# jay-tux/cutrace

Measured on AMD Instinct MI355X. Metric: Mrays/sec (primary+secondary), higher is better.
Workload: dtype f32; 1 GPU; bunny.json@1920x1080 bounces=5 fudge=1e-3, 1 frame(s)/step row-tiled over 1 GPU(s), gather to rank 0; steps_in_flight=1

## Files before the change

cutrace_amd/__init__.py:

```python
import contextlib
import ctypes as C
import os

import numpy as np

from . import _lib
from ._lib import Camera, Light, Material, Object, RenderStats, Rows, SceneDesc, Triangle, Vec3

ROOT = _lib.ROOT

VAR_AUTO = 0
VAR_NO_PREFILTER = 2
VAR_NO_ANYHIT = 4
VAR_NO_CLUSTER = 8
VAR_STATS = 16
VAR_EXACT_POW = 32
VAR_NO_REORDER = 256
VAR_NO_OCC6 = 512
VAR_NO_DIRECT = 1024
VAR_IMAGE_ORDER_FIRST = 2048
VAR_MERGE = 4096
VAR_IGNORE_TRANSPARENT = 8192

RAY_IGNORE_TRANSPARENT = 1
# ... 166 lines not shown
            st = L.ctr_render(self._h, C.c_float(fudge), bounces, C.byref(r), depth.ctypes.data, color.ctypes.data,
                              normal.ctypes.data, C.byref(stats))
            if st:
                raise RuntimeError(f"ctr_render failed ({st}): {L.ctr_last_error().decode()}")
        return dict(depth=depth, color=color, normal=normal, ray_count=int(stats.ray_count),
                    kernel_ms=stats.kernel_ms, total_ms=stats.total_ms, max_depth=float(stats.max_depth),
                    rows=int(stats.rows))

    def render_uv(self, fudge=1e-3, bounces=5, rows=None):
        L = _lib.hip_lib()
        r = make_rows(self.h, rows)
        n = rows_count(self.h, rows)
        depth = np.empty((n, self.w), np.float32)
        color = np.empty((n, self.w, 3), np.float32)
        normal = np.empty((n, self.w, 3), np.float32)
        uv = np.empty((n, self.w, 2), np.float32)
        stats = RenderStats()
        st = L.ctr_render_uv(self._h, C.c_float(fudge), bounces, C.byref(r), depth.ctypes.data, color.ctypes.data,
                             normal.ctypes.data, uv.ctypes.data, C.byref(stats))
        if st:
            raise RuntimeError(f"ctr_render_uv failed ({st}): {L.ctr_last_error().decode()}")
        return dict(depth=depth, color=color, normal=normal, uv=uv, ray_count=int(stats.ray_count),
                    kernel_ms=stats.kernel_ms, total_ms=stats.total_ms, max_depth=float(stats.max_depth), rows=int(stats.rows))

    def render_device(self, d_depth, d_color, d_normal, d_counters=0, stream=0, fudge=1e-3, bounces=5, rows=None, samples=1):
        samples = self._samples(samples)
        L = _lib.hip_lib()
        r = make_rows(self.h, rows)
        if samples != 1:
            st = L.ctr_render_device_aa(self._h, C.c_float(fudge), bounces, samples, C.byref(r), d_depth, d_color, d_normal,
                                        d_counters, stream)
            if st:
                raise RuntimeError(f"ctr_render_device_aa failed ({st}): {L.ctr_last_error().decode()}")
            return
        st = L.ctr_render_device(self._h, C.c_float(fudge), bounces, C.byref(r), d_depth, d_color, d_normal,
                                 d_counters, stream)
        if st:
            raise RuntimeError(f"ctr_render_device failed ({st}): {L.ctr_last_error().decode()}")

    def set_cameras(self, cams):
        arr = (Camera * len(cams))(*cams)
        st = _lib.hip_lib().ctr_scene_set_cameras(self._h, arr, len(cams))
        if st:
            raise RuntimeError(f"ctr_scene_set_cameras failed: {_lib.hip_lib().ctr_last_error().decode()}")
        self.n_cams = len(cams)

    def render_device_batch(self, d_depth, d_color, d_normal, n_frames, frame_stride_px, first_frame=0, d_counters=0,
                            stream=0, fudge=1e-3, bounces=5, rows=None, part_stride=0):
        L = _lib.hip_lib()
        r = make_rows(self.h, rows)
        st = L.ctr_render_device_batch(self._h, C.c_float(fudge), bounces, C.byref(r), first_frame, n_frames,
                                       frame_stride_px, part_stride, d_depth, d_color, d_normal, d_counters, stream)
        if st:
            raise RuntimeError(f"ctr_render_device_batch failed ({st}): {L.ctr_last_error().decode()}")

    def algorithmic_bytes(self, fudge=1e-3, bounces=5, rows=None):
        L = _lib.hip_lib()
        r = make_rows(self.h, rows)
        b = C.c_uint64()
        n = C.c_uint64()
        st = L.ctr_algorithmic_bytes(self._h, C.c_float(fudge), bounces, C.byref(r), C.byref(b), C.byref(n))
        if st:
            raise RuntimeError(f"ctr_algorithmic_bytes failed ({st}): {L.ctr_last_error().decode()}")
        return int(b.value), int(n.value)

    def last_counters(self):
        out = np.zeros(16, np.uint64)
        _lib.hip_lib().ctr_last_counters(self._h, out.ctypes.data)
        return out

    @staticmethod
    def lane_stats(reset=True):
        raw = np.zeros(96, np.uint64)
        if _lib.hip_lib().ctr_debug_lane_stats(raw.ctypes.data, 1 if reset else 0):
            raise RuntimeError("ctr_debug_lane_stats failed")
        c = [int(x) for x in raw]
        trips, live = c[72], c[73]
        out = {"wave_trips": trips, "live_lanes_per_trip": live / trips if trips else None,
               "live_fraction": live / (64.0 * trips) if trips else None,
               "live_fraction_of_in_image_lanes": (live / trips) / (c[75] / c[74]) if trips and c[74] and c[75] else None,
               "trips_by_live_lanes_1_8_to_57_64": c[64:72], "trips_mixing_kinds": c[76], "waves": c[74],
               "merged_walks": c[78], "merged_walks_redone": c[77],
               "shadow_casts_at_meshes": {"wave_casts": c[80], "receivers_all_off_mesh": c[81], "of_those_unoccluded_by_meshes": c[82],
                                          "unoccluded_by_meshes_any_receiver": c[83]}}
        kinds = {}
        for d in range(16):
            for name, base in (("radiance", 0), ("shadow", 16)):
                if c[32 + base + d]:
                    label = "primary" if (name == "radiance" and d == 0) else f"{name}@depth{d}"
                    kinds[label] = {"lanes": c[base + d], "trips": c[32 + base + d],
                                    "lanes_per_trip": c[base + d] / c[32 + base + d]}
        out["by_kind"] = kinds
        return out

    def _torch_device(self):
        import torch
        return torch.device("cuda", self.device)

    def _rays_arg(self, x, what, cols):
        import torch
        dev = self._torch_device()
        if isinstance(x, torch.Tensor):
            if x.device.type != "cpu" and x.device != dev:
                raise ValueError(f"{what}: tensor on {x.device}, the scene lives on {dev}")
        elif isinstance(x, np.ndarray):
            x = torch.from_numpy(x)
        else:
            raise TypeError(f"{what}: expected a torch tensor or a numpy array, got {type(x).__name__}")
        shape_ok = x.dim() == 1 if cols == 0 else (x.dim() == 2 and x.shape[1] == cols)
        if x.dtype != torch.float32 or not shape_ok:
            raise ValueError(f"{what}: expected float32 of shape {'(n,)' if cols == 0 else f'(n, {cols})'}, "
                             f"got {x.dtype} {tuple(x.shape)}")
        return x.to(dev, non_blocking=False).contiguous()

    def _cast(self, q, keep, stream):
        import torch
        q.n_rays = keep[0].shape[0]
        q.d_origin, q.d_dir = keep[0].data_ptr() or None, keep[1].data_ptr() or None
        st = _lib.hip_lib().ctr_cast_rays(self._h, C.byref(q), C.c_void_p(stream.cuda_stream))
        if st:
            raise RuntimeError(f"ctr_cast_rays failed ({st}): {_lib.hip_lib().ctr_last_error().decode()}")

    def _per_ray(self, x, n, what):
        if isinstance(x, (int, float, np.integer, np.floating)):
            return float(x), None
        v = self._rays_arg(x, what, 0)
        if v.shape[0] != n:
            raise ValueError(f"{what}: {v.shape[0]} values for {n} rays")
        return 0.0, v

    def cast_rays(self, origins, dirs, min_t=1e-3, ignore_transparent=False, linear=False, outputs=None, stream=None):
        import torch
        outputs = RAY_OUTPUTS if outputs is None else tuple(outputs)
        bad = [k for k in outputs if k not in RAY_OUTPUTS]
        if bad or not outputs:
            raise ValueError(f"outputs: a non-empty subset of {RAY_OUTPUTS}, got {outputs}")
        dev = self._torch_device()
        with torch.cuda.device(dev), torch.cuda.stream(stream if stream is not None else torch.cuda.current_stream(dev)):
            o = self._rays_arg(origins, "origins", 3)
            d = self._rays_arg(dirs, "dirs", 3)
            n = o.shape[0]
            if d.shape[0] != n:
                raise ValueError(f"dirs: {d.shape[0]} rays for {n} origins")
            q = _lib.RayQuery()
            q.flags = (RAY_IGNORE_TRANSPARENT if ignore_transparent else 0) | (RAY_LINEAR if linear else 0)
            q.min_t, mt = self._per_ray(min_t, n, "min_t")
            q.d_min_t = mt.data_ptr() if mt is not None and n else None
            shapes = {"t": ((n,), torch.float32), "object": ((n,), torch.int32), "prim": ((n,), torch.int32),
                      "point": ((n, 3), torch.float32), "normal": ((n, 3), torch.float32), "uv": ((n, 2), torch.float32)}
            out = {k: torch.empty(*shapes[k][0], dtype=shapes[k][1], device=dev) for k in outputs}
            for k, v in out.items():
                setattr(q, "d_" + k, v.data_ptr() if n else None)
            if n:
                self._cast(q, (o, d, mt), torch.cuda.current_stream(dev))
        return out

    def shadow(self, origins, dirs, max_t, linear=False, stream=None):
        import torch
        dev = self._torch_device()
        with torch.cuda.device(dev), torch.cuda.stream(stream if stream is not None else torch.cuda.current_stream(dev)):
            o = self._rays_arg(origins, "origins", 3)
            d = self._rays_arg(dirs, "dirs", 3)
            n = o.shape[0]
            if d.shape[0] != n:
                raise ValueError(f"dirs: {d.shape[0]} rays for {n} origins")
            q = _lib.RayQuery()
            q.flags = RAY_SHADOW | (RAY_LINEAR if linear else 0)
# ... 171 lines not shown
```

cutrace_amd/csrc/render_kernel.hip:

```cpp
#include <hip/hip_runtime.h>
#include <math.h>
#include <stddef.h>
#include <stdint.h>
#include <stdlib.h>

#include "cutrace_amd.h"
#include "scene_device.h"
#include "bvh.h"

#define CADDR __attribute__((address_space(4)))
#define BALLOT(p) __builtin_amdgcn_ballot_w64(p)
#define HIDE_UNIFORM(x) asm volatile("" : "+v"(x))
#define PIN3(a, b, c) asm volatile("" : "+v"(a), "+v"(b), "+v"(c))
#define INVB(m) __builtin_amdgcn_inverse_ballot_w64(m)
#define FCMP(a, b, pred) __builtin_amdgcn_fcmpf((a), (b), (pred))
enum { FC_OEQ = 1, FC_OGT = 2, FC_OGE = 3, FC_OLT = 4, FC_OLE = 5 };
#define TL_NONE 0x7FFFFFFFu

extern "C" __device__ uint32_t ctr_writelane(uint32_t value, uint32_t lane, uint32_t old) __asm("llvm.amdgcn.writelane.i32");

namespace {

#if defined(CTR_PROFILE)
__device__ unsigned int g_prof[128];
// ... 372 lines not shown
        atomicAdd(&g_lane_stats[64 + ((n_live - 1u) >> 3)], 1ull);
        atomicAdd(&g_lane_stats[72], 1ull);
        atomicAdd(&g_lane_stats[73], (unsigned long long)n_live);
        if (kinds > 1u) atomicAdd(&g_lane_stats[76], 1ull);
        if (first_trip) { atomicAdd(&g_lane_stats[74], 1ull); atomicAdd(&g_lane_stats[75], (unsigned long long)__builtin_popcountll(img_m)); }
      }
    }

    float best = INFINITY;
    int bobj = -1, btri = -1;
    mask_t alive_m = active_m;
    V3 rinv = mk(0, 0, 0);
    bool have_rinv = false;
    V3 ria = mk(0, 0, 0);
    float ria_big = 0.f;
    float cmax = 0.f;
    if (k_has_mesh) {
      CTR_MARK(2);
      ria = mk(fminf(fmaxf(__builtin_amdgcn_rcpf(rd.x), -1e30f), 1e30f),
               fminf(fmaxf(__builtin_amdgcn_rcpf(rd.y), -1e30f), 1e30f),
               fminf(fmaxf(__builtin_amdgcn_rcpf(rd.z), -1e30f), 1e30f));
      ria_big = fmaxf(fmaxf(fabsf(ria.x), fabsf(ria.y)), fabsf(ria.z));
      cmax = fmaxf(fmaxf(fabsf(rd.x), fabsf(rd.y)), fabsf(rd.z));
    }

    TSTAMP(t_loop0);
    TACC(0, t_trip0, t_loop0);
    CTR_MARK(3);
    const bool anyhit_cast = ANYHIT && shadow_cast;
    const bool ign_now = IGNTR && first_trip;
    {
      mask_t live_m = alive_m;
      const float mt_lo = min_t - fabsf(min_t) * 0x1p-21f;
      float lhv = anyhit_cast ? light_dist : best;
      lhv = lhv + fabsf(lhv) * 0x1p-21f;
      float tiny = 1e-37f;
      asm volatile("" : "+v"(tiny));
      auto plane_exact = [&](uint32_t pidx, float num, float den, mask_t need_m, auto site) -> bool {
        CTR_MARK(110 + decltype(site)::value);
        bool retire = false;
        if (INVB(need_m)) {
          const float t0 = num / den;
          if (__builtin_isfinite(t0) && t0 > min_t) {
            if (t0 < best || (t0 == best && (int)pidx < bobj)) {
              best = t0; bobj = (int)pidx; btri = -1;
              if (!anyhit_cast) lhv = t0 + fabsf(t0) * 0x1p-21f;
            }
            if (anyhit_cast && t0 < light_dist) retire = true;
          }
        }
        if (ANYHIT) {
          live_m &= ~BALLOT(retire);
          if (live_m == 0ull) return false;
        }
        return true;
      };
      auto plane_test = [&](uint32_t pidx, float num, float den, auto site) -> bool {
        CTR_MARK(100 + decltype(site)::value);
        const float nump = __uint_as_float(__float_as_uint(num) ^ (__float_as_uint(den) & 0x80000000u));
        const float denp = fabsf(den);
        const mask_t need_m = live_m & ~(FCMP(nump, __builtin_fmaf(mt_lo, denp, -tiny), FC_OLT) |
                                         FCMP(nump, __builtin_fmaf(lhv, denp, tiny), FC_OGT));
        if (need_m == 0ull) return true;
        return plane_exact(pidx, num, den, need_m, site);
      };
      const float2_ rox = {ro.x, ro.x}, roy = {ro.y, ro.y}, roz = {ro.z, ro.z};
      const float2_ rdx = {rd.x, rd.x}, rdy = {rd.y, rd.y}, rdz = {rd.z, rd.z};
      auto num_den = [&](const CADDR DPlanePair &P, float2_ &num, float2_ &den) {
        const float2_ nx = ldpair(P.n[0]), ny = ldpair(P.n[1]), nz = ldpair(P.n[2]);
        const float2_ dx = ldpair(P.p[0]) - rox, dy = ldpair(P.p[1]) - roy, dz = ldpair(P.p[2]) - roz;
        num = (dx * nx + dy * ny) + dz * nz;
        den = (rdx * nx + rdy * ny) + rdz * nz;
      };
      const uint32_t n_recs = k_plane_recs, n_axis = k_axis_recs;
      bool axis_fast = false;
      if (n_axis != 0u && A.fudge >= 1e-30f) {
        CTR_MARK(4);
        const float chk = __builtin_fmaf(ro.x, 4.0f, __builtin_fmaf(ro.y, 4.0f, __builtin_fmaf(ro.z, 4.0f, (rd.x + rd.y) + rd.z))) * 0.0f;
        axis_fast = (alive_m & ~FCMP(chk, 0.0f, FC_OEQ)) == 0ull;
      }
      auto triple_tests = [&](uint32_t i00, uint32_t i01, uint32_t i10, uint32_t i11, uint32_t i20, uint32_t i21, float2_ num0, float2_ den0,
                              float2_ num1, float2_ den1, float2_ num2, float2_ den2, uint32_t tr00, uint32_t tr01, uint32_t tr10,
                              uint32_t tr11, uint32_t tr20, uint32_t tr21) -> bool {
        if (i00 != CTR_PLANE_PAD && !(IGNTR && ign_now && tr00)) { if (!plane_test(i00, num0.x, den0.x, SITE(0))) return false; }
        if (i01 != CTR_PLANE_PAD && !(IGNTR && ign_now && tr01)) { if (!plane_test(i01, num0.y, den0.y, SITE(1))) return false; }
        if (i10 != CTR_PLANE_PAD && !(IGNTR && ign_now && tr10)) { if (!plane_test(i10, num1.x, den1.x, SITE(2))) return false; }
        if (i11 != CTR_PLANE_PAD && !(IGNTR && ign_now && tr11)) { if (!plane_test(i11, num1.y, den1.y, SITE(3))) return false; }
        if (i20 != CTR_PLANE_PAD && !(IGNTR && ign_now && tr20)) { if (!plane_test(i20, num2.x, den2.x, SITE(4))) return false; }
        if (i21 != CTR_PLANE_PAD && !(IGNTR && ign_now && tr21)) { if (!plane_test(i21, num2.y, den2.y, SITE(5))) return false; }
        return true;
      };
      uint32_t p = 0;
      bool more = true;
      if (k_head_axis && axis_fast) {
        CTR_MARK(59);
        auto pr = [&](int k) -> float2_ { const float2_ v = {__uint_as_float(hd_ax[2 * k]), __uint_as_float(hd_ax[2 * k + 1])}; return v; };
        const float2_ nx = pr(1), ny = pr(3), nz = pr(5);
        uint32_t tr00 = 0u, tr01 = 0u, tr10 = 0u, tr11 = 0u, tr20 = 0u, tr21 = 0u;
        if (IGNTR && ign_now) {
          tr00 = AK->head.ax_transparent[0]; tr01 = AK->head.ax_transparent[1]; tr10 = AK->head.ax_transparent[2];
          tr11 = AK->head.ax_transparent[3]; tr20 = AK->head.ax_transparent[4]; tr21 = AK->head.ax_transparent[5];
        }
        p = 3u;
        more = triple_tests(hd_ax[12], hd_ax[13], hd_ax[14], hd_ax[15], hd_ix[0], hd_ix[1], (pr(0) - rox) * nx, rdx * nx, (pr(2) - roy) * ny,
                            rdy * ny, (pr(4) - roz) * nz, rdz * nz, tr00, tr01, tr10, tr11, tr20, tr21);
      }
      while (more && p < n_recs) {
        if (n_recs - p >= 3u) {
          float2_ num0, den0, num1, den1, num2, den2;
          uint32_t i00, i01, i10, i11, i20, i21;
          uint32_t tr00 = 0u, tr01 = 0u, tr10 = 0u, tr11 = 0u, tr20 = 0u, tr21 = 0u;
          const CADDR DPlanePair &P0 = k_planes[p], &P1 = k_planes[p + 1], &P2 = k_planes[p + 2];
          i00 = P0.index[0]; i01 = P0.index[1]; i10 = P1.index[0]; i11 = P1.index[1]; i20 = P2.index[0]; i21 = P2.index[1];
          if (IGNTR && ign_now) {
            tr00 = P0.transparent[0]; tr01 = P0.transparent[1]; tr10 = P1.transparent[0];
            tr11 = P1.transparent[1]; tr20 = P2.transparent[0]; tr21 = P2.transparent[1];
          }
          if (p < n_axis && axis_fast) {
            CTR_MARK(5);
            const float2_ nx = ldpair(P0.n[0]), ny = ldpair(P1.n[1]), nz = ldpair(P2.n[2]);
            num0 = (ldpair(P0.p[0]) - rox) * nx; den0 = rdx * nx;
            num1 = (ldpair(P1.p[1]) - roy) * ny; den1 = rdy * ny;
            num2 = (ldpair(P2.p[2]) - roz) * nz; den2 = rdz * nz;
          } else {
            CTR_MARK(6);
            num_den(P0, num0, den0);
            num_den(P1, num1, den1);
            num_den(P2, num2, den2);
          }
          p += 3;
          if (!triple_tests(i00, i01, i10, i11, i20, i21, num0, den0, num1, den1, num2, den2, tr00, tr01, tr10, tr11, tr20, tr21)) break;
        } else {
          const CADDR DPlanePair &P0 = k_planes[p];
          CTR_MARK(7);
          float2_ num0, den0;
          num_den(P0, num0, den0);
          const uint32_t i00 = P0.index[0], i01 = P0.index[1];
          p += 1;
          if (!(IGNTR && ign_now && P0.transparent[0])) { if (!plane_test(i00, num0.x, den0.x, SITE(6))) break; }
          if (i01 != CTR_PLANE_PAD && !(IGNTR && ign_now && P0.transparent[1])) {
            if (!plane_test(i01, num0.y, den0.y, SITE(7))) break;
          }
        }
      }
      if (ANYHIT) alive_m = live_m;
    }
    TSTAMP(t_planes1);
    TACC(1, t_loop0, t_planes1);
    CTR_MARK(8);
    V3 sph_d = mk(0, 0, 0);
    float sph_dd = 0.f;
    bool sph_have = false;
    for (uint32_t oi = 0; oi < k_n_oloop; ++oi) {
      if (ANYHIT) {
        if (alive_m == 0ull) break;
      }
      const CADDR DObj &O = AK->oloop[oi];
      const uint32_t i = O.index;
      const uint32_t type = O.type;
      if (IGNTR && ign_now && __float_as_uint(O.f[7]) != 0u) continue;
      CTR_MARK(9);
      bool ok = false;
      float cand = INFINITY;
      int ctri = -1;
      if (type == CTR_OBJ_SPHERE) {
        if (!sph_have) {
// ... 480 lines not shown
          } else {
            for (uint32_t k = 0; k < cnt; ++k) {
              tri_test(load_tri(A.tris[beg + k]), beg + k, bb_m);
              if (ANYHIT) {
                if (bb_m == 0ull) break;
              }
            }
          }
          if (STATS) {
            for (int off = 32; off > 0; off >>= 1) {
              const uint32_t on = (uint32_t)__shfl_xor((int)pl_nodes, off), ot = (uint32_t)__shfl_xor((int)pl_tris, off);
              pl_nodes = on > pl_nodes ? on : pl_nodes;
              pl_tris = ot > pl_tris ? ot : pl_tris;
            }
            st[9] += (uint32_t)__builtin_amdgcn_readfirstlane((int)pl_nodes);
            st[10] += (uint32_t)__builtin_amdgcn_readfirstlane((int)pl_tris);
          }
          int i_lane = merged ? 0 : (int)i;
          int ctri_lane = (int)(beg + morig);
          if (MERGE && merged) {
            CTR_MARK(86);
            if (STATS && lane == 0) atomicAdd(&g_lane_stats[78], 1ull);
            mask_t todo = BALLOT(morig != 0xFFFFFFFFu);
            mask_t bad_m = BALLOT(mt != INFINITY && !(mt > min_t));
            while (todo != 0ull) {
              const uint32_t rk = (uint32_t)__builtin_amdgcn_readlane((int)morig, (int)__builtin_ctzll(todo)) >> 24;
              const mask_t same_m = todo & BALLOT((morig >> 24) == rk);
              const CADDR DObj &R = AK->meshes[k_mesh + 1u + rk];
              const uint32_t r_index = R.index, r_beg = R.tri_begin;
              bad_m |= same_m & ~box_test(R, same_m, SITE(1));
              if (INVB(same_m)) { i_lane = (int)r_index; ctri_lane = (int)(r_beg + (morig & 0xFFFFFFu)); }
              todo &= ~same_m;
            }
            if (bad_m != 0ull) {
              CTR_MARK(87);
              if (STATS && lane == 0) atomicAdd(&g_lane_stats[77], 1ull);
              if (ANYHIT) {
                alive_m |= bad_m & anyhit_m;
                if (INVB(anyhit_m & ~alive_m)) { best = fminf(0.5f * light_dist, 1e30f); bobj = i_lane; }
              }
              t_pend = AK->tlas_root2;
              t_sp = 0u;
              continue;
            }
          }
          CTR_MARK(35);
          if (ANYHIT) {
            if (INVB(anyhit_m & ~alive_m)) { best = fminf(0.5f * light_dist, 1e30f); bobj = i_lane; }
          }
          ok = mt != INFINITY;
          cand = mt;
          ctri = ctri_lane;
          obj_lane = i_lane;
#ifdef CTR_TIMING
          {
            const unsigned long long t_mesh1 = __builtin_readcyclecounter();
            if (t_w0 == 0) t_w0 = t_bb;
            tm[5] += (t_mesh1 - t_w0) - t_leaves;
            tm[6] += t_leaves;
          }
#endif

        }
        if (INVB(alive_m) && ok && cand > min_t && (cand < best || (cand == best && obj_lane < bobj))) {
          best = cand;
          bobj = obj_lane;
          btri = ctri;
        }
      }
    }
    if (STATS && st_shadow_entry != 0ull && lane == 0) {
      const bool planes_only = (st_recv_mesh & st_shadow_entry) == 0ull, none_occluded = (st_shadow_entry & ~alive_m) == 0ull;
      atomicAdd(&g_lane_stats[80], 1ull);
      if (planes_only) atomicAdd(&g_lane_stats[81], 1ull);
      if (planes_only && none_occluded) atomicAdd(&g_lane_stats[82], 1ull);
      if (none_occluded) atomicAdd(&g_lane_stats[83], 1ull);
    }
    const bool was_hit = bobj >= 0;
    TSTAMP(t_loop1);
    CTR_MARK(36);

    typedef uint32_t u32x4 __attribute__((ext_vector_type(4)));
    const u32x8 cold = *(const CADDR u32x8 *)&AK->objs;
    const u32x4 cold2 = *(const CADDR u32x4 *)&AK->n_light;
    const CADDR DObj *const k_objs = (const CADDR DObj *)(((uint64_t)cold[1] << 32) | cold[0]);
    const CADDR float *const k_gnorm = (const CADDR float *)(((uint64_t)cold[3] << 32) | cold[2]);
    const CADDR DLight *const k_lights = (const CADDR DLight *)(((uint64_t)cold[5] << 32) | cold[4]);
    const CADDR DMat *const k_mats = (const CADDR DMat *)(((uint64_t)cold[7] << 32) | cold[6]);
    const uint32_t k_n_light = cold2[0];
    const int k_bounces = (int)cold2[1];
    int act = ACT_NONE;
    float first_depth = 0.f;
    uint32_t nl_type = 0u;
    V3 nl_v = mk(0.f, 0.f, 0.f);
    if (MSP_IS_RADIANCE(msp)) {
      const V3 ro_keep = ro;
      V3 normal = mk(0, 0, 0);
      float tc_u = 0.0f, tc_v = 0.0f;
      if (was_hit) {
        const CADDR DObj &H = k_objs[bobj];
        CTR_MARK(37);
        const uint32_t ht = H.type;
        const float hf0 = H.f[0], hf1 = H.f[1], hf2 = H.f[2], hf3 = H.f[3], hf4 = H.f[4], hf5 = H.f[5];
        float gn0 = 0.f, gn1 = 0.f, gn2 = 0.f;
        if (btri >= 0) { gn0 = k_gnorm[4 * btri + 0]; gn1 = k_gnorm[4 * btri + 1]; gn2 = k_gnorm[4 * btri + 2]; }
        mat_i = H.mat;
        if (STATS) recv_mesh = (ht == CTR_OBJ_MESH || ht == CTR_OBJ_TRIANGLE);
        { const CADDR DLight &L0 = k_lights[0]; nl_type = L0.type; nl_v = mk(L0.vx, L0.vy, L0.vz); }
        pos = vadd(ro, vscale(in_d, best));
        float unused_n0;
        const V3 hit_dn = vnormalized_n(in_d, unused_n0);
        CTR_MARK(92);
        set_in_dn(hit_dn);
        if (ht == CTR_OBJ_SPHERE) {
          CTR_MARK(38);
          const V3 hit = vadd(ro, vscale(hit_dn, best));
          normal = vnormalized(vsub(hit, mk(hf0, hf1, hf2)));
          ro = hit;
          if (UV && first_trip) {
            tc_u = 0.5f + (atan2f(normal.z, normal.x) / (2.0f * (float)M_PI));
            tc_v = 0.5f + (asinf(normal.y) / (float)M_PI);
          }
        } else if (ht == CTR_OBJ_PLANE) {
          ro = pos;
          normal = mk(hf3, hf4, hf5);
          if (UV && first_trip) {
            const V3 ax1 = vnormalized(mk(normal.y, -normal.x, 0.0f));
            const V3 ax2 = vcross(normal, ax1);
            const V3 mod_pt = vsub(mk(hf0, hf1, hf2), pos);
            tc_u = vdot(ax1, mod_pt);
            tc_v = vdot(ax2, mod_pt);
          }
        } else {
          ro = pos;
          normal = mk(gn0, gn1, gn2);
          if (UV && first_trip) {
            if (ht == CTR_OBJ_MESH) {
              tc_u = pos.x;
              tc_v = pos.y;
            } else {
              const CADDR DTri &T = A.tris[btri];
              const V3 p1 = mk(hf0, hf1, hf2), p2 = mk(T.px, T.py, T.pz), p3 = mk(hf3, hf4, hf5);
              const V3 p2p1 = vsub(p2, p1), p3p1 = vsub(p3, p1), xp1 = vsub(pos, p1);
              const V3 proj_u = vscale(p2p1, vdot(xp1, p2p1) / vdot(p2p1, p2p1));
              const V3 proj_v = vscale(p3p1, vdot(xp1, p3p1) / vdot(p3p1, p3p1));
              tc_u = vnorm(proj_u) / vnorm(p2p1);
              tc_v = vnorm(proj_v) / vnorm(p3p1);
            }
          }
        }
      }
      CTR_MARK(39);
      if (first_trip) {
        CTR_MARK(40);
        const size_t px_id = px_index();
        float *const k_depth_out = ((const CADDR KParams *)AK)->depth_out, *const k_normal_out = ((const CADDR KParams *)AK)->normal_out;
        if constexpr (SS) {
          if (ss_kept()) {
            k_depth_out[px_id] = best;
            store3(k_normal_out, px_id, normal);
          }
        } else {
          if (HOSTOUT) __hip_atomic_store(k_depth_out + px_id, best, __ATOMIC_RELAXED, __HIP_MEMORY_SCOPE_AGENT);
          else k_depth_out[px_id] = best;
          store3(k_normal_out, px_id, normal);
        }
        if (UV) {
          float *const uvp = AK->uv_out;
          uvp[2 * px_id + 0] = tc_u;
          uvp[2 * px_id + 1] = tc_v;
        }
        first_depth = best;
      }
      CTR_MARK(41);
      if (IGNTR && ign_now) {
        ro = ro_keep;
        min_t = A.fudge;
      } else if (!was_hit) {
        out_rgb = mk(0.f, 0.f, 0.f);
        act = ACT_UNWIND;
      } else {
        CTR_MARK(42);
        const CADDR DMat &M = k_mats[mat_i];
        fin = vscale(mk(M.cx, M.cy, M.cz), ambient);
        { float unused_n; const V3 nrm_ = vnormalized_n(normal, unused_n); CTR_MARK(93); set_nn(nrm_); }
        li = 0;
        act = ACT_LIGHT;
      }
    } else if (MSP_IS_SHADOW(msp)) {
      CTR_MARK(43);
      { const CADDR DLight &L1 = k_lights[li + 1u]; nl_type = L1.type; nl_v = mk(L1.vx, L1.vy, L1.vz); }
      bool done_shadow;
      float shadow_fac = 0.f;
      if (was_hit && best < light_dist) {
        const float trans = ANYHIT ? 0.0f : k_mats[k_objs[bobj].mat].transparency;
        if (!ANYHIT) intensity += (1.0f - trans);
        if (ANYHIT || intensity >= 1.0f) { shadow_fac = 1.0f; done_shadow = true; }
        else {
          min_t = (float)((double)best + 1e-3);
          done_shadow = false;
        }
      } else {
        shadow_fac = ANYHIT ? 0.0f : intensity;
        done_shadow = true;
      }
      if (done_shadow) {
        if (shadow_fac < 1.0f) {
          CTR_MARK(44);
          const CADDR DMat &M = k_mats[mat_i];
          const CADDR DLight &Lg = k_lights[li];
          const V3 diffuse = mk(M.cx, M.cy, M.cz);
          const V3 specular = vscale(diffuse, M.specular);
          const V3 color = mk(Lg.cx, Lg.cy, Lg.cz);
          const V3 nd = rd;
          const V3 nn_ = get_nn();
          const float fd = smax(0.0f, vdot(nn_, nd));
          const V3 ld = vmul(diffuse, color);
          const V3 hsum = vadd(vscale(get_in_dn(), -1.0f), nd);
          const V3 hv = FASTPOW ? vscale(hsum, __builtin_amdgcn_rsqf(vdot(hsum, hsum))) : vnormalized(hsum);
          const float sx = smax(0.0f, vdot(nn_, hv));
          float fs;
          if (FASTPOW) {
            fs = (M.phong_exp == 0.0f) ? 1.0f : __builtin_amdgcn_exp2f(M.phong_exp * __builtin_amdgcn_logf(sx));
          } else {
            fs = (float)pow((double)sx, (double)M.phong_exp);
          }
          const V3 ls = vmul(specular, color);
          fin = vadd(fin, vscale(vadd(vscale(ld, fd), vscale(ls, fs)), 1 - shadow_fac));
        }
        CTR_MARK(45);
        li++;
        act = ACT_LIGHT;
      }
    }

    TSTAMP(t_cont_mid);
    TACC(7, t_loop1, t_cont_mid);
    CTR_MARK(46);
    if (act == ACT_LIGHT) {
      if (li < k_n_light) {
        CTR_MARK(47);
        const uint32_t lg_type = nl_type;
        const V3 lg_v = nl_v;
        V3 direction;
        float distance;
        if (lg_type == CTR_LIGHT_SUN) {
          direction = vscale(lg_v, -1.0f);
          distance = INFINITY;
        } else {
          CTR_MARK(48);
          const V3 diff = vsub(lg_v, ro);
          direction = vnormalized_n(diff, distance);
          CTR_MARK(94);
        }
        CTR_MARK(49);
        float dir_norm;
        rd = vnormalized_n(direction, dir_norm);
        CTR_MARK(95);
        light_dist = distance * dir_norm;
        intensity = 0.0f;
        min_t = (float)(0.0 + 1e-3);
        msp |= MSP_SHADOW;
      } else {
        act = ACT_BOUNCE;
      }
    }

    if (act == ACT_BOUNCE) {
      CTR_MARK(50);
      const CADDR DMat &M = k_mats[mat_i];
      const float reflective = M.reflexivity, translucent = M.transparency;
      const int sp = MSP_DEPTH(msp);
      const bool more = sp < k_bounces;
      const bool do_refl = more && (double)reflective >= 1e-6;
      const bool do_trans = more && (double)translucent >= 1e-6;
      if (do_refl || do_trans) {
        CTR_MARK(51);
        STK(sp, F_R) = fin.x; STK(sp, F_G) = fin.y; STK(sp, F_B) = fin.z;
        STK(sp, F_MAT) = __uint_as_float(mat_i | (do_refl ? 1u << 30 : 2u << 30));
        if (do_refl && do_trans) {
          CTR_MARK(96);
          STK(sp, F_PX) = pos.x; STK(sp, F_PY) = pos.y; STK(sp, F_PZ) = pos.z;
          STK(sp, F_DX) = in_d.x; STK(sp, F_DY) = in_d.y; STK(sp, F_DZ) = in_d.z;
        }
        CTR_MARK(120);
        msp = (uint32_t)(sp + 1);
        if (do_refl) {
          const V3 nn_ = get_nn(), dn_ = get_in_dn();
          in_d = vsub(dn_, vscale(nn_, 2.0f * vdot(nn_, dn_)));
        }
        ro = pos; rd = in_d;
        min_t = A.fudge;
      } else {
        out_rgb = fin;
        act = ACT_UNWIND;
      }
    }

    if (act == ACT_UNWIND) {
      int sp = MSP_DEPTH(msp);
      for (;;) {
        CTR_MARK(52);
        if (sp == 0) {
          if constexpr (SS) {
            STK(0, F_R) = out_rgb.x; STK(0, F_G) = out_rgb.y; STK(0, F_B) = out_rgb.z;
            msp = MSP_DONE | 1u;
          } else {
            const size_t px_id = px_index();
            store3(((const CADDR KParams *)AK)->color_out, px_id, out_rgb);
            msp = MSP_DONE;
          }
          break;
        }
        CTR_MARK(53);
        --sp;
        V3 rgb = mk(STK(sp, F_R), STK(sp, F_G), STK(sp, F_B));
// ... 609 lines not shown
```

cutrace_amd/csrc/scene_device.h:

```cpp
#ifndef CUTRACE_AMD_SCENE_DEVICE_H
#define CUTRACE_AMD_SCENE_DEVICE_H

#include <stddef.h>
#include <stdint.h>

struct DTri {
  float ab[3][2];
  float px, py, pz;
  uint32_t orig;
  float nx, ny, nz;
  float ke;
  float ke2;
  float pad1;
};
static_assert(sizeof(DTri) == 64, "DTri must be one 64-byte line");

#define CTR_OBJ_MERGED 4u
#define CTR_MERGE_MAX_MESHES 255u
struct DObj {
  uint32_t type;
  uint32_t mat;
  uint32_t tri_begin;
  uint32_t tri_count;
  uint32_t node_begin;
  uint32_t node_count;
  uint32_t bvh_root;
  uint32_t index;
  float f[8];
};
static_assert(sizeof(DObj) == 64, "DObj must be 64 bytes");

struct DPlanePair {
  float p[3][2];
  float n[3][2];
  uint32_t index[2];
  uint32_t transparent[2];
};
static_assert(sizeof(DPlanePair) == 64, "DPlanePair must be 64 bytes");
#define CTR_PLANE_PAD 0xFFFFFFFFu

struct DLight {
  uint32_t type;
  float vx, vy, vz;
  float cx, cy, cz;
  float pad;
};
static_assert(sizeof(DLight) == 32, "DLight must be 32 bytes");

struct DMat {
  float cx, cy, cz;
  float specular, reflexivity, phong_exp, transparency;
  float pad;
};
static_assert(sizeof(DMat) == 32, "DMat must be 32 bytes");

struct DCam {
  float pos[3], up[3], forward[3], right[3];
  float ambient;
  uint32_t w, h;
};

enum : uint32_t {
  KV_PREFILTER = 1u,
  KV_ANYHIT = 2u,
  KV_COUNT = 4u,
  KV_BVH = 8u,
  KV_STATS = 16u,
  KV_FASTPOW = 32u,
  KV_OCC6 = 64u,
  KV_HOSTOUT = 128u,
  KV_UV = 256u,
  KV_IGNTR = 1024u,
  KV_MERGE = 512u,
  KV_SS = 2048u,
};

struct DRows {
  uint32_t row_begin;
  uint32_t row_end;
  uint32_t part_stride;
  uint32_t n_rows;
  uint32_t block_rows;
  uint32_t part, n_parts;
  uint32_t first_block;
};

struct alignas(64) DSceneHead {
  float ax[6][2];
  uint32_t ax_index[6];
  uint32_t ax_transparent[6];
  uint32_t n_axis_recs;
  uint32_t n_mesh;
  uint32_t pad[6];
  DObj mesh;
};
static_assert(sizeof(DSceneHead) == 192 && offsetof(DSceneHead, mesh) == 128, "DSceneHead: two 64-byte lines of planes, one of mesh");
#define CTR_TL_HEAD_FLAG 0x40000000u

struct RenderLaunch {
  const DObj *objs;
  const DObj *oloop;
  const DObj *meshes;
  uint32_t n_mesh, tlas_root, tlas_begin;
  uint32_t tlas_root_regular;
  float tl_mn[3], tl_mx[3];
  const DPlanePair *planes;
  uint32_t n_oloop, n_plane_recs, n_axis_recs;
  const DTri *tris;
  const void *nodes;
  const void *nodes4;
  const float *gnorm;
  const DLight *lights;
  const DMat *mats;
  uint32_t n_obj, n_light, n_mat;
  uint32_t has_mesh;
  uint32_t need_cold_frames;
  uint32_t any_bounce;
  const DCam *cams;
  uint32_t w, h;
  uint32_t first_frame, n_frames;
  uint64_t frame_stride_px;
  DRows rows;
  float fudge;
  int bounces;
  float *depth;
  float *color;
  float *normal;
  float *uv;
  unsigned long long *shards;
  unsigned long long *counters;
  uint32_t variant;
  const uint32_t *order;
  uint32_t *cost;
  uint32_t *order_next;
  uint32_t order_init;
  float *host_depth, *host_color, *host_normal;
  uint32_t *group_done;
  uint32_t ss_log2;
  DSceneHead head;
};
uint64_t ctr_staging_pixels(const RenderLaunch &L);
uint64_t ctr_staging_groups(const RenderLaunch &L);
uint32_t ctr_group_tile_count(const RenderLaunch &L, uint64_t group);
uint64_t ctr_staging_index(const RenderLaunch &L, uint32_t x, uint32_t k_row);
bool ctr_host_delivery_available(uint32_t kernel_variant);

void ctr_internal_set_error(const char *msg);
int ctr_launch_render(const RenderLaunch &L, void *stream);
uint64_t ctr_launch_waves(const RenderLaunch &L);
#define CTR_SHARDS 1024
#define CTR_SHARD_WORDS 16
#define CTR_COST_BINS 1024u
#define CTR_MAX_BOUNCES 15

#endif
```

cutrace_amd/csrc/scene_flatten.cpp:

```cpp
#include "scene_flatten.h"

#include <algorithm>
#include <atomic>
#include <chrono>
#include <cmath>
#include <cstdio>
#include <cstdlib>
#include <cstring>
#include <thread>

namespace {

constexpr float KAPPA = 1.0f / 16384.0f;

struct f3 { float x, y, z; };
inline f3 sub(ctr_vec3 a, ctr_vec3 b) { return {a.x - b.x, a.y - b.y, a.z - b.z}; }
inline f3 cross(f3 a, f3 o) { return {a.y * o.z - a.z * o.y, a.z * o.x - a.x * o.z, a.x * o.y - a.y * o.x}; }

void make_tri(const ctr_vec3 &p1, const ctr_vec3 &p2, const ctr_vec3 &p3, uint32_t orig, DTri &T, float *gn) {
  f3 a = sub(p2, p1), b = sub(p2, p3);
  T.ab[0][0] = a.x; T.ab[1][0] = a.y; T.ab[2][0] = a.z;
  T.ab[0][1] = b.x; T.ab[1][1] = b.y; T.ab[2][1] = b.z;
  T.px = p2.x; T.py = p2.y; T.pz = p2.z;
  f3 n = cross(a, b);
// ... 333 lines not shown
  if (d.n_objects > 0xFFFFFFFFull || d.n_triangles > 0x7FFFFFFFull || d.cam.w > 0x7FFFFFFFull ||
      d.cam.h > 0x7FFFFFFFull)
    return bad("scene too large for 32-bit device indices");
  if (d.cam.w * d.cam.h > 0x7FFFFFFFull * 2) return bad("image too large");
  for (uint64_t i = 0; i < d.n_objects; i++) {
    const ctr_object &o = d.objects[i];
    if (o.type > CTR_OBJ_SPHERE) return bad("object #" + std::to_string(i) + ": bad type");
    if (o.mat_idx >= d.n_materials) return bad("object #" + std::to_string(i) + ": material index out of range");
    if (o.type == CTR_OBJ_MESH && (o.tri_begin > d.n_triangles || o.tri_count > d.n_triangles - o.tri_begin))
      return bad("object #" + std::to_string(i) + ": triangle range out of bounds");
  }
  for (uint64_t i = 0; i < d.n_lights; i++)
    if (d.lights[i].type > CTR_LIGHT_POINT) return bad("light #" + std::to_string(i) + ": bad type");
  for (uint64_t i = 0; i < d.n_materials; i++)
    if (d.materials[i].type != CTR_MAT_PHONG) return bad("material #" + std::to_string(i) + ": bad type");
  return CTR_OK;
}

int flatten_scene(const ctr_scene_desc &d, FlatScene &F, std::string &err) {
  F = FlatScene();
  if (int st = object_records(d, mesh_trees(d), F, err)) return st;
  create_stamp("meshes: BVH + records");
  plane_records(F);
  const std::vector<DObj> in_scene_order = nonempty_meshes(F);
  top_level(in_scene_order, F);
  reserve_merged(d, in_scene_order, F);
  lights_and_materials(d, F);
  for (const MeshGuard &g : F.guards) F.mesh_tris += g.tri_count;
  F.mesh_bytes = F.tris.size() * sizeof(DTri) + F.nodes.size() * sizeof(DNode) + F.nodes4.size() * sizeof(DNode4);
  F.ray_slots = ray_stack_slots(F);
  create_stamp("planes, top level, materials");
  return CTR_OK;
}

std::vector<DirtyRange> build_merged_tree(FlatScene &F) {
  Merged &M = F.merged;
  if (!M.reserved || M.built) return {};
  const uint32_t total = M.tri_count, n_rank = (uint32_t)M.slot_of.size() - 1;
  std::vector<uint32_t> rank_of(total);
  for (uint32_t r = 0; r < n_rank; r++)
    for (uint32_t k = M.slot_of[r]; k < M.slot_of[r + 1]; k++) rank_of[k] = r;
  std::vector<DNode4> mnodes;
  std::vector<uint32_t> order;
  bvh4_build(tri_boxes(M.src.data(), total), BVH_LEAF, mnodes, order);
  if (mnodes.size() > M.node_cap) return {};
  M.node_count = (uint32_t)mnodes.size();
  std::copy(mnodes.begin(), mnodes.end(), F.nodes4.begin() + M.node_begin);
  M.where.assign(total, 0u);
  float dummy_gn[4];
  for (uint32_t k = 0; k < total; k++) {
    const uint32_t g = order[k], r = rank_of[g], f = g - M.slot_of[r];
    const ctr_triangle &t = M.src[g];
    make_tri(t.p1, t.p2, t.p3, (r << 24) | f, F.tris[M.tri_begin + k], dummy_gn);
    M.where[g] = k;
  }
  for (uint32_t k = 0; k < CTR_GUARD_SLOTS; k++) F.tris[M.tri_begin + total + k] = F.tris[M.tri_begin];
  DObj &P = F.meshes[F.n_mesh];
  P.node_count = M.node_count;
  P.bvh_root = 0;
  M.built = true;
  M.guarded.assign(1, 0xFFFFFFFFu);
  return {{DirtyRange::TRIS, M.tri_begin, (size_t)total + CTR_GUARD_SLOTS, {}},
          {DirtyRange::NODES4, M.node_begin, M.node_count, {}},
          {DirtyRange::MESHES, F.n_mesh, 1, {}}};
}

void fill_scene_head(const FlatScene &F, uint32_t tlas_root, DSceneHead &H) {
  H = DSceneHead{};
  if (F.n_axis_recs >= 3u && F.planes.size() >= 3u) {
    for (int r = 0; r < 3; r++)
      for (int k = 0; k < 2; k++) {
        H.ax[2 * r][k] = F.planes[r].p[r][k];
        H.ax[2 * r + 1][k] = F.planes[r].n[r][k];
        H.ax_index[2 * r + k] = F.planes[r].index[k];
        H.ax_transparent[2 * r + k] = F.planes[r].transparent[k];
      }
    H.n_axis_recs = 3u;
  }
  const uint32_t leaf = tlas_root & 0xFFFFFFu;
  if (F.n_mesh != 0u && (tlas_root & BVH_LEAF_FLAG) && leaf < F.meshes.size()) {
    H.mesh = F.meshes[leaf];
    H.n_mesh = 1u;
  }
}
```

Measured before the change: 72680 Mrays/s.

## Cache lights and materials in kernel-arg head and add wave-wide shadow plane gate

Copies small light and material tables into the kernel-argument scene head, so shadow shading can read them as wave-uniform scalar loads when every shadow lane shares the same light and material. Also adds a ballot-based pre-test in the plane triple check for all-shadow waves: if every live lane is outside all six planes, the per-plane tests are skipped. The aim is to cut vector memory loads and divergent plane tests on shadow rays. In exchange the kernel-argument struct grows, register pressure rises from the duplicated shading path, and a stats counter is added.

```diff
diff --git a/cutrace_amd/__init__.py b/cutrace_amd/__init__.py
--- a/cutrace_amd/__init__.py
+++ b/cutrace_amd/__init__.py
@@ -272,7 +272,8 @@
                "trips_by_live_lanes_1_8_to_57_64": c[64:72], "trips_mixing_kinds": c[76], "waves": c[74],
                "merged_walks": c[78], "merged_walks_redone": c[77],
                "shadow_casts_at_meshes": {"wave_casts": c[80], "receivers_all_off_mesh": c[81], "of_those_unoccluded_by_meshes": c[82],
-                                          "unoccluded_by_meshes_any_receiver": c[83]}}
+                                          "unoccluded_by_meshes_any_receiver": c[83]},
+               "shadow_trips": {"scalar": c[84], "vector": c[85]}}
         kinds = {}
         for d in range(16):
             for name, base in (("radiance", 0), ("shadow", 16)):
diff --git a/cutrace_amd/csrc/render_kernel.hip b/cutrace_amd/csrc/render_kernel.hip
--- a/cutrace_amd/csrc/render_kernel.hip
+++ b/cutrace_amd/csrc/render_kernel.hip
@@ -478,6 +478,36 @@
       auto triple_tests = [&](uint32_t i00, uint32_t i01, uint32_t i10, uint32_t i11, uint32_t i20, uint32_t i21, float2_ num0, float2_ den0,
                               float2_ num1, float2_ den1, float2_ num2, float2_ den2, uint32_t tr00, uint32_t tr01, uint32_t tr10,
                               uint32_t tr11, uint32_t tr20, uint32_t tr21) -> bool {
+#ifndef CTR_NO_TRIPLE_GATE
+#ifdef CTR_TRIPLE_GATE_ALWAYS
+        if (true) {
+#else
+        if (ANYHIT && (live_m & ~shadow_m) == 0ull) {
+#endif
+          CTR_MARK(127);
+          auto out_m = [&](float num, float den) -> mask_t {
+            const float nump = __uint_as_float(__float_as_uint(num) ^ (__float_as_uint(den) & 0x80000000u));
+            const float denp = fabsf(den);
+            return FCMP(nump, __builtin_fmaf(mt_lo, denp, -tiny), FC_OLT) | FCMP(nump, __builtin_fmaf(lhv, denp, tiny), FC_OGT);
+          };
+          mask_t all_out;
+          if (IGNTR) {
+            auto slot = [&](uint32_t idx, uint32_t tr, float num, float den) -> mask_t {
+              return (idx == CTR_PLANE_PAD || (ign_now && tr)) ? ~0ull : out_m(num, den);
+            };
+            all_out = slot(i00, tr00, num0.x, den0.x) & slot(i01, tr01, num0.y, den0.y) & slot(i10, tr10, num1.x, den1.x) &
+                      slot(i11, tr11, num1.y, den1.y) & slot(i20, tr20, num2.x, den2.x) & slot(i21, tr21, num2.y, den2.y);
+          } else {
+            auto rec = [&](uint32_t idx0, float2_ num, float2_ den) -> mask_t {
+              mask_t o = out_m(num.x, den.x) & out_m(num.y, den.y);
+              asm volatile("" : "+s"(o));
+              return idx0 == CTR_PLANE_PAD ? ~0ull : o;
+            };
+            all_out = rec(i00, num0, den0) & rec(i10, num1, den1) & rec(i20, num2, den2);
+          }
+          if ((live_m & ~all_out) == 0ull) return true;
+        }
+#endif
         if (i00 != CTR_PLANE_PAD && !(IGNTR && ign_now && tr00)) { if (!plane_test(i00, num0.x, den0.x, SITE(0))) return false; }
         if (i01 != CTR_PLANE_PAD && !(IGNTR && ign_now && tr01)) { if (!plane_test(i01, num0.y, den0.y, SITE(1))) return false; }
         if (i10 != CTR_PLANE_PAD && !(IGNTR && ign_now && tr10)) { if (!plane_test(i10, num1.x, den1.x, SITE(2))) return false; }
@@ -1124,13 +1154,36 @@
 
     typedef uint32_t u32x4 __attribute__((ext_vector_type(4)));
     const u32x8 cold = *(const CADDR u32x8 *)&AK->objs;
-    const u32x4 cold2 = *(const CADDR u32x4 *)&AK->n_light;
+    const u32x2 cold2 = *(const CADDR u32x2 *)&AK->n_light;
     const CADDR DObj *const k_objs = (const CADDR DObj *)(((uint64_t)cold[1] << 32) | cold[0]);
     const CADDR float *const k_gnorm = (const CADDR float *)(((uint64_t)cold[3] << 32) | cold[2]);
     const CADDR DLight *const k_lights = (const CADDR DLight *)(((uint64_t)cold[5] << 32) | cold[4]);
     const CADDR DMat *const k_mats = (const CADDR DMat *)(((uint64_t)cold[7] << 32) | cold[6]);
     const uint32_t k_n_light = cold2[0];
     const int k_bounces = (int)cold2[1];
+    bool sc_shadow = false;
+    DLight sc_lg = {}, sc_l1 = {};
+    DMat sc_m = {};
+#ifndef CTR_NO_SCALAR_SHADOW
+    if (ANYHIT && shadow_m != 0ull) {
+      const uint32_t first = (uint32_t)__builtin_ctzll(shadow_m);
+      const uint32_t li0 = __builtin_amdgcn_readlane(li, first), mat0 = __builtin_amdgcn_readlane(mat_i, first);
+      const u32x2 held = *(const CADDR u32x2 *)&AK->head.n_lights;
+      const uint32_t li_c = li0 < CTR_HEAD_LIGHTS ? li0 : CTR_HEAD_LIGHTS - 1u, mat_c = mat0 & (CTR_HEAD_MATS - 1u);
+      u32x8 r_lg = *(const CADDR u32x8 *)&AK->head.lights[li_c];
+      u32x8 r_l1 = *(const CADDR u32x8 *)&AK->head.lights[li_c + 1u];
+      u32x8 r_m = *(const CADDR u32x8 *)&AK->head.mats[mat_c];
+      const bool uniform = (shadow_m & ~(BALLOT(li == li0) & BALLOT(mat_i == mat0))) == 0ull;
+      asm volatile("" : "+s"(r_lg), "+s"(r_l1), "+s"(r_m));
+      sc_shadow = uniform && li0 < held[0] && mat0 < held[1];
+      sc_lg = DLight{r_lg[0], __uint_as_float(r_lg[1]), __uint_as_float(r_lg[2]), __uint_as_float(r_lg[3]), __uint_as_float(r_lg[4]),
+                     __uint_as_float(r_lg[5]), __uint_as_float(r_lg[6]), 0.f};
+      sc_l1 = DLight{r_l1[0], __uint_as_float(r_l1[1]), __uint_as_float(r_l1[2]), __uint_as_float(r_l1[3]), 0.f, 0.f, 0.f, 0.f};
+      sc_m = DMat{__uint_as_float(r_m[0]), __uint_as_float(r_m[1]), __uint_as_float(r_m[2]), __uint_as_float(r_m[3]), 0.f,
+                  __uint_as_float(r_m[5]), 0.f, 0.f};
+    }
+#endif
+    if (STATS && shadow_m != 0ull && lane == 0) atomicAdd(&g_lane_stats[sc_shadow ? 84 : 85], 1ull);
     int act = ACT_NONE;
     float first_depth = 0.f;
     uint32_t nl_type = 0u;
@@ -1230,50 +1283,63 @@
         act = ACT_LIGHT;
       }
     } else if (MSP_IS_SHADOW(msp)) {
-      CTR_MARK(43);
-      { const CADDR DLight &L1 = k_lights[li + 1u]; nl_type = L1.type; nl_v = mk(L1.vx, L1.vy, L1.vz); }
-      bool done_shadow;
-      float shadow_fac = 0.f;
-      if (was_hit && best < light_dist) {
-        const float trans = ANYHIT ? 0.0f : k_mats[k_objs[bobj].mat].transparency;
-        if (!ANYHIT) intensity += (1.0f - trans);
-        if (ANYHIT || intensity >= 1.0f) { shadow_fac = 1.0f; done_shadow = true; }
-        else {
-          min_t = (float)((double)best + 1e-3);
-          done_shadow = false;
-        }
+#define CTR_SHADOW_STEP(NEXT, MAT, LIGHT, ID43, ID44)                                                             \
+      CTR_MARK(ID43);                                                                                             \
+      { const auto &L1 = (NEXT); nl_type = L1.type; nl_v = mk(L1.vx, L1.vy, L1.vz); }                             \
+      bool done_shadow;                                                                                           \
+      float shadow_fac = 0.f;                                                                                     \
+      if (was_hit && best < light_dist) {                                                                         \
+                           \
+        const float trans = ANYHIT ? 0.0f : k_mats[k_objs[bobj].mat].transparency;                                \
+        if (!ANYHIT) intensity += (1.0f - trans);                                                                 \
+        if (ANYHIT || intensity >= 1.0f) { shadow_fac = 1.0f; done_shadow = true; }                               \
+        else {                                                                                                    \
+          min_t = (float)((double)best + 1e-3);              \
+          done_shadow = false;                                                         \
+        }                                                                                                         \
+      } else {                                                                                                    \
+        shadow_fac = ANYHIT ? 0.0f : intensity;    \
+        done_shadow = true;                                                                                       \
+      }                                                                                                           \
+      if (done_shadow) {                                                                                          \
+        if (shadow_fac < 1.0f) {                                                                                  \
+                                                                                           \
+          CTR_MARK(ID44);                                                                    \
+          const auto &M = (MAT);                                                                                  \
+          const auto &Lg = (LIGHT);                                                                               \
+          const V3 diffuse = mk(M.cx, M.cy, M.cz);                                                                \
+          const V3 specular = vscale(diffuse, M.specular);                            \
+          const V3 color = mk(Lg.cx, Lg.cy, Lg.cz);                                                               \
+          const V3 nd = rd;              \
+          const V3 nn_ = get_nn();                                                                                \
+          const float fd = smax(0.0f, vdot(nn_, nd));                                                             \
+          const V3 ld = vmul(diffuse, color);                                                                     \
+          const V3 hsum = vadd(vscale(get_in_dn(), -1.0f), nd);                                                   \
+                        \
+                                      \
+          const V3 hv = FASTPOW ? vscale(hsum, __builtin_amdgcn_rsqf(vdot(hsum, hsum))) : vnormalized(hsum);      \
+          const float sx = smax(0.0f, vdot(nn_, hv));                                                             \
+          float fs;                                                                                               \
+          if (FASTPOW) {                                                                                          \
+                           \
+                            \
+            fs = (M.phong_exp == 0.0f) ? 1.0f : __builtin_amdgcn_exp2f(M.phong_exp * __builtin_amdgcn_logf(sx));  \
+          } else {                                                                                                \
+            fs = (float)pow((double)sx, (double)M.phong_exp);    \
+          }                                                                                                       \
+          const V3 ls = vmul(specular, color);                                                                    \
+          fin = vadd(fin, vscale(vadd(vscale(ld, fd), vscale(ls, fs)), 1 - shadow_fac));                          \
+        }                                                                                                         \
+        CTR_MARK(45);                                                                                             \
+        li++;                                                                                                     \
+        act = ACT_LIGHT;                                                                                          \
+      }
+      if (ANYHIT && sc_shadow) {
+        CTR_SHADOW_STEP(sc_l1, sc_m, sc_lg, 84, 85)
       } else {
-        shadow_fac = ANYHIT ? 0.0f : intensity;
-        done_shadow = true;
+        CTR_SHADOW_STEP(k_lights[li + 1u], k_mats[mat_i], k_lights[li], 43, 44)
       }
-      if (done_shadow) {
-        if (shadow_fac < 1.0f) {
-          CTR_MARK(44);
-          const CADDR DMat &M = k_mats[mat_i];
-          const CADDR DLight &Lg = k_lights[li];
-          const V3 diffuse = mk(M.cx, M.cy, M.cz);
-          const V3 specular = vscale(diffuse, M.specular);
-          const V3 color = mk(Lg.cx, Lg.cy, Lg.cz);
-          const V3 nd = rd;
-          const V3 nn_ = get_nn();
-          const float fd = smax(0.0f, vdot(nn_, nd));
-          const V3 ld = vmul(diffuse, color);
-          const V3 hsum = vadd(vscale(get_in_dn(), -1.0f), nd);
-          const V3 hv = FASTPOW ? vscale(hsum, __builtin_amdgcn_rsqf(vdot(hsum, hsum))) : vnormalized(hsum);
-          const float sx = smax(0.0f, vdot(nn_, hv));
-          float fs;
-          if (FASTPOW) {
-            fs = (M.phong_exp == 0.0f) ? 1.0f : __builtin_amdgcn_exp2f(M.phong_exp * __builtin_amdgcn_logf(sx));
-          } else {
-            fs = (float)pow((double)sx, (double)M.phong_exp);
-          }
-          const V3 ls = vmul(specular, color);
-          fin = vadd(fin, vscale(vadd(vscale(ld, fd), vscale(ls, fs)), 1 - shadow_fac));
-        }
-        CTR_MARK(45);
-        li++;
-        act = ACT_LIGHT;
-      }
+#undef CTR_SHADOW_STEP
     }
 
     TSTAMP(t_cont_mid);
diff --git a/cutrace_amd/csrc/scene_device.h b/cutrace_amd/csrc/scene_device.h
--- a/cutrace_amd/csrc/scene_device.h
+++ b/cutrace_amd/csrc/scene_device.h
@@ -85,16 +85,23 @@
   uint32_t first_block;
 };
 
+#define CTR_HEAD_LIGHTS 4u
+#define CTR_HEAD_MATS 8u
 struct alignas(64) DSceneHead {
   float ax[6][2];
   uint32_t ax_index[6];
   uint32_t ax_transparent[6];
   uint32_t n_axis_recs;
   uint32_t n_mesh;
-  uint32_t pad[6];
+  uint32_t n_lights;
+  uint32_t n_mats;
+  uint32_t pad[4];
   DObj mesh;
+  DLight lights[CTR_HEAD_LIGHTS + 1u];
+  DMat mats[CTR_HEAD_MATS];
 };
-static_assert(sizeof(DSceneHead) == 192 && offsetof(DSceneHead, mesh) == 128, "DSceneHead: two 64-byte lines of planes, one of mesh");
+static_assert(offsetof(DSceneHead, mesh) == 128 && offsetof(DSceneHead, lights) == 192 && offsetof(DSceneHead, mats) == 352 && sizeof(DSceneHead) == 640,
+              "DSceneHead: two 64-byte lines of planes, one of mesh, the light and material tables on 32-byte boundaries");
 #define CTR_TL_HEAD_FLAG 0x40000000u
 
 struct RenderLaunch {
diff --git a/cutrace_amd/csrc/scene_flatten.cpp b/cutrace_amd/csrc/scene_flatten.cpp
--- a/cutrace_amd/csrc/scene_flatten.cpp
+++ b/cutrace_amd/csrc/scene_flatten.cpp
@@ -439,4 +439,10 @@
     H.mesh = F.meshes[leaf];
     H.n_mesh = 1u;
   }
-}
+  if (!F.lights.empty() && F.lights.size() <= CTR_HEAD_LIGHTS && !F.mats.empty() && F.mats.size() <= CTR_HEAD_MATS) {
+    for (size_t i = 0; i < F.lights.size(); i++) H.lights[i] = F.lights[i];
+    for (size_t i = 0; i < F.mats.size(); i++) H.mats[i] = F.mats[i];
+    H.n_lights = (uint32_t)F.lights.size();
+    H.n_mats = (uint32_t)F.mats.size();
+  }
+}
```

Result: slower. 70170 Mrays/s (-3.5%).
